# ColumbiaDVMM/ColumbiaImageSearch

Measured on AMD Instinct MI355X. Metric: queries/sec @ recall@10 on 10M LOPQ index, higher is better.
Workload: dtype f64

## Files before the change

columbiaimagesearch_amd/csrc/lopq_scan3.hip:

```cpp
#include "scan_common.h"
#include <cmath>
#include <cstdio>
#include <cstdlib>

typedef unsigned short u16x2_t __attribute__((ext_vector_type(2)));

static __device__ __forceinline__ uint32_t pk_add_u16(uint32_t a, uint32_t b) {
    return __builtin_bit_cast(uint32_t, (u16x2_t)(__builtin_bit_cast(u16x2_t, a) + __builtin_bit_cast(u16x2_t, b)));
}
static __device__ __forceinline__ uint32_t pk_subsat_u16(uint32_t a, uint32_t b) {
    return __builtin_bit_cast(uint32_t, __builtin_elementwise_sub_sat(__builtin_bit_cast(u16x2_t, a), __builtin_bit_cast(u16x2_t, b)));
}

static __device__ __forceinline__ uint32_t pk_min_u16(uint32_t a, uint32_t b) {
    return __builtin_bit_cast(uint32_t, __builtin_elementwise_min(__builtin_bit_cast(u16x2_t, a), __builtin_bit_cast(u16x2_t, b)));
}

static const int S3G = 4;

#ifdef CIS_S3_COUNTERS
__device__ unsigned long long g_s3_ctr[16];
#define S3_CLK() ((long long)__builtin_amdgcn_s_memtime())
#define S3_CTR(i, v) do { if (threadIdx.x == 0) atomicAdd(&g_s3_ctr[i], (unsigned long long)(v)); } while (0)
extern "C" int cis_debug_counters3(unsigned long long* out, int reset) {
// ... 557 lines not shown
                const uint32_t sg = (g & 1) ? (d[u][g >> 1] >> 16) : (d[u][g >> 1] & 0xffffu);
                const uint32_t t1 = (g & 1) ? ((g >> 1) ? s23 >> 16 : s01 >> 16) : ((g >> 1) ? s23 & 0xffffu : s01 & 0xffffu);
                pm[u][g] = __ballot(sg < t1) & anym[u];
                if (any_dup) {
                    bool same = true;
#pragma unroll
                    for (int i = 0; i < (M + 3) / 4; ++i) same = same && (cur[u].w[i] == dup[g].w[i]);
                    pm[u][g] &= ~(__ballot(same) & (has_dup[g] ? ~0ull : 0ull));
                }
            }
        }
#pragma unroll
        for (int g = 0; g < G; ++g) {
            if (g >= ng) break;
            uint32_t* rk = rk_all + (g * NW + w) * R;
            int ntot = 0;
#pragma unroll
            for (int u = 0; u < U; ++u) ntot += __popcll(pm[u][g]);
            if (ntot == 0) continue;
            auto entry = [&](int u) -> uint32_t {
                const uint32_t sg = (g & 1) ? (d[u][g >> 1] >> 16) : (d[u][g >> 1] & 0xffffu);
                return (sg << 16) | (uint32_t)(base + u * 64 + lane);
            };
            if (cnt[g] + ntot <= R) {
                int c = cnt[g];
#pragma unroll
                for (int u = 0; u < U; ++u) {
                    const unsigned long long m = pm[u][g];
                    if (m == 0ull) continue;
                    const int idx = __builtin_amdgcn_mbcnt_hi((unsigned)(m >> 32), __builtin_amdgcn_mbcnt_lo((unsigned)m, c));
                    if ((m >> lane) & 1ull) rk[idx] = entry(u);
                    c += __popcll(m);
                }
                cnt[g] = c;
                continue;
            }
            int u0 = 0;
            while (true) {
                bool full = false;
#pragma unroll
                for (int u = 0; u < U; ++u) {
                    const unsigned long long m = pm[u][g];
                    if (u < u0 || full || m == 0ull) continue;
                    const int n = __popcll(m);
                    if (cnt[g] + n > R) {
                        full = true;
                        u0 = u;
                        continue;
                    }
                    const int idx = cnt[g] + __builtin_amdgcn_mbcnt_hi((unsigned)(m >> 32), __builtin_amdgcn_mbcnt_lo((unsigned)m, 0));
                    if ((m >> lane) & 1ull) rk[idx] = entry(u);
                    cnt[g] += n;
                    u0 = u + 1;
                }
                if (!full) break;
                const QScale qsg = load_scale(&sh[g]);
                int c2 = wave_compact3<M, NR, NW>(rk, cnt[g], L, Lw, R - 64, qsg, &sh[g], w);
                if (c2 < 0) {
                    uint32_t dp = 0xffffffffu;
                    const WorkItem itg = items[item_idx[g]];
                    c2 = wave_compact3_exact<M, NR, NW>(rk, cnt[g], L, Lw, qsg, &sh[g], w, codes, start, K,
                                                        T + (int64_t)itg.tab0 * nf * K, T + (int64_t)itg.tab1 * nf * K, dp);
                    dp = (uint32_t)__builtin_amdgcn_readfirstlane((int)dp);
                    if (dp != 0xffffffffu) {
                        dup[g] = load_code<M>(codes, start + (int64_t)dp);
                        has_dup[g] = true;
                        any_dup = true;
                    }
                }
                cnt[g] = c2;
                const uint32_t thg = lds_ld(&sh[g].thr);
                if (lane == 0) st16(&thr1[g], thg + 1u);
                const unsigned long long dup_on = has_dup[g] ? ~0ull : 0ull;
#pragma unroll
                for (int u = 0; u < U; ++u) {
                    const uint32_t sg = (g & 1) ? (d[u][g >> 1] >> 16) : (d[u][g >> 1] & 0xffffu);
                    bool same = true;
#pragma unroll
                    for (int i = 0; i < (M + 3) / 4; ++i) same = same && (cur[u].w[i] == dup[g].w[i]);
                    pm[u][g] &= __ballot(sg <= thg) & ~(__ballot(same) & dup_on);
                }
            }
        }
    }
    S3_CTR(4, S3_CLK() - c0);
#pragma unroll
    for (int g = 0; g < G; ++g) {
        if (g >= ng) break;
        uint32_t* rk = rk_all + (g * NW + w) * R;
        if (cnt[g] > 0) cnt[g] = wave_compact3<M, NR, NW>(rk, cnt[g], L, Lw, NR * 64, load_scale(&sh[g]), &sh[g], w);
    }
    S3_CTR(5, S3_CLK() - c0);
    if constexpr (NW > 1) __syncthreads();
    S3_CTR(6, S3_CLK() - c0);
#pragma unroll
    for (int g = 0; g < G; ++g) {
        if (g >= ng) break;
        uint32_t* rk = rk_all + (g * NW + w) * R;
        const QScale qsg = load_scale(&sh[g]);
        if constexpr (NW > 1) cnt[g] = wave_filter3<NR, NW>(rk, cnt[g], qsg, &sh[g]);
        if (lane == 0) sh[g].wcnt[w] = cnt[g];
        if (tid == 0) {
            const uint64_t b = block_bound<NW>(&sh[g]);
            if (b < sh[g].ext) atomicMin(&qbound[items[item_idx[g]].q], (unsigned long long)b);
        }
    }
    if constexpr (NW > 1) __syncthreads();
#pragma unroll
    for (int g = 0; g < G; ++g) {
        if (g >= ng) break;
        const uint32_t* rk = rk_all + (g * NW + w) * R;
        int off = 0, total = 0;
#pragma unroll
        for (int i = 0; i < NW; ++i) {
            const int c = (NW > 1) ? sh[g].wcnt[i] : cnt[g];
            off += (i < w) ? c : 0;
            total += c;
        }
        uint64_t* out = item_surv + (int64_t)item_idx[g] * S + off;
        for (int e = lane; e < cnt[g]; e += 64) {
            const uint32_t x = rk[e];
            out[e] = ((uint64_t)(x >> 16) << 32) | (x & 0xffffu);
        }
        if (tid == 0) item_n[item_idx[g]] = total;
    }
    S3_CTR(7, S3_CLK() - c0);
    S3_CTR(0, 1);
}

template <int M, int NR, int U, int NW, int WPE>
__global__ __launch_bounds__(NW * 64) __attribute__((amdgpu_waves_per_eu(WPE, WPE))) void k_adc_scan3(
    const WorkItem* __restrict__ items, const TabDesc* __restrict__ tabs, const int* __restrict__ slots,
    const int* __restrict__ n_slots_ptr, const double* __restrict__ T, const float* __restrict__ T32,
    const uint8_t* __restrict__ codes, int K, int L, int S, int* __restrict__ queue_ctr ,
    uint64_t* __restrict__ item_surv, int* __restrict__ item_n, float* __restrict__ item_slack,
    unsigned long long* __restrict__ qbound , int two_pass, int single_queue ) {
    extern __shared__ __attribute__((aligned(16))) char smem[];
    constexpr int G = S3G;
    constexpr int R = NR * 64 - 8;
    int* s_next = reinterpret_cast<int*>(smem + (size_t)K * M * G * 2 + (size_t)G * NW * R * 4 + G * sizeof(Scan3Shared) + 32);
    const int* qs = n_slots_ptr + 8;
    const int home = blockIdx.x & 7;
    const long long k0 = S3_CLK();
    (void)k0;
    for (int a = 0; a < 8; ++a) {
        const int x = (home + a) & 7;
        const int qstart = qs[x];
        const int count = single_queue ? (x == 0 ? qs[1] - qstart : 0) : qs[x + 1] - qstart;
        if (count <= 0) continue;
        while (true) {
            const long long q0 = S3_CLK();
            (void)q0;
            int j;
            if constexpr (NW > 1) {
                __syncthreads();
                if (threadIdx.x == 0) *s_next = atomicAdd(&queue_ctr[x], 1);
                __syncthreads();
                j = __builtin_amdgcn_readfirstlane(*s_next);
            } else {
                int t = 0;
                if (threadIdx.x == 0) t = atomicAdd(&queue_ctr[x], 1);
                j = __builtin_amdgcn_readfirstlane(t);
            }
            S3_CTR(8, S3_CLK() - q0);
            if (j >= count) break;
            const int slot = qstart + j;
            int idx[G];
            int ng = 0;
            bool same = true;
#pragma unroll
            for (int g = 0; g < G; ++g) {
                idx[g] = slots[slot * G + g];
                if (idx[g] >= 0) {
                    ng = g + 1;
                    same = same && items[idx[g]].start == items[idx[0]].start && items[idx[g]].len == items[idx[0]].len;
                } else {
                    idx[g] = idx[0];
                }
            }
            if (!same) {
                for (int g2 = 0; g2 < ng; ++g2) {
                    int oi[G];
#pragma unroll
                    for (int g = 0; g < G; ++g) {
                        oi[g] = idx[0];
#pragma unroll
                        for (int gg = 1; gg < G; ++gg)
                            if (gg == g2) oi[g] = idx[gg];
                    }
                    if (g2 > 0) __syncthreads();
                    scan3_group<M, NR, U, NW>(items, tabs, oi, 1, T, T32, codes, K, L, S, item_surv, item_n, item_slack, qbound, smem, two_pass != 0);
                }
                continue;
            }
            scan3_group<M, NR, U, NW>(items, tabs, idx, ng, T, T32, codes, K, L, S, item_surv, item_n, item_slack, qbound, smem, two_pass != 0);
        }
    }
    S3_CTR(9, S3_CLK() - k0);
    S3_CTR(10, 1);
}

struct Slot4 {
    int item[S3G], tab0[S3G], tab1[S3G], q[S3G];
    float qinv[S3G];
    int start_lo, start_hi, len, ng;
    int ist_lo[S3G], ist_hi[S3G], ilen[S3G];
};
struct Scan4Shared {
    double inv_up, ub;
    uint64_t ext;
    uint32_t tau;
    int verify;
    int cnt;
    int q;
};

template <int M, int UU, int OCT = (M >= 8 ? 8 : 4), bool TWO = false>
__device__ __forceinline__ void adc16_rows(const CodeWords<M> (&cur)[UU], const RotConsts<M>& rc, const Adc16Consts<M, TWO>& gc,
                                           u32x2_t (&d)[UU]) {
    constexpr int NU = M / OCT;
    u32x2_t fbuf[2][OCT];
    uint32_t D[2][(M + 3) / 4];
    rot_words<M>(cur[0], rc, D[0]);
    adc16_issue<M, OCT, TWO>(D[0], 0, gc, fbuf[0]);
#pragma unroll
    for (int q = 0; q < UU * NU; ++q) {
        const int u = q / NU, o = q % NU;
        if (q + 1 < UU * NU) {
            const int u1 = (q + 1) / NU, o1 = (q + 1) % NU;
            if (o1 == 0) rot_words<M>(cur[u1], rc, D[u1 & 1]);
            adc16_issue<M, OCT, TWO>(D[u1 & 1], o1, gc, fbuf[(q + 1) & 1]);
        }
        __builtin_amdgcn_sched_barrier(0);
        const u32x2_t part = adc16_sum<OCT>(fbuf[q & 1]);
        if (o == 0) {
            d[u] = part;
        } else {
            d[u][0] = pk_add_u16(d[u][0], part[0]);
            d[u][1] = pk_add_u16(d[u][1], part[1]);
        }
        __builtin_amdgcn_sched_barrier(0);
    }
}

static __device__ __forceinline__ void lds_barrier() {
    asm volatile("s_waitcnt lgkmcnt(0)\n\ts_barrier" ::: "memory");
}

#ifndef CIS_S4_U
#define CIS_S4_U 2
#endif
#ifndef CIS_S4_UL
#define CIS_S4_UL 2
#endif
#ifndef CIS_S4_OCT
#define CIS_S4_OCT 4
#endif
#ifndef CIS_S4_WPE
#define CIS_S4_WPE 6
#endif
static const int S4_OCT = CIS_S4_OCT;
#ifndef CIS_S4_PF
#define CIS_S4_PF 2
#endif
#ifndef CIS_S4_LCAP
#define CIS_S4_LCAP 504
#endif
#ifndef CIS_S4_NS
#define CIS_S4_NS 16
#endif
#ifndef CIS_S4_Z
#define CIS_S4_Z 4.0f
#endif
static const int S4_DS = 8;
static const int S4_LCAP = CIS_S4_LCAP;
static const int S4_NS = CIS_S4_NS;

static const int S4_LCAP_LONG = 1016;

static const int S4_TWO_NRP = 24;
static constexpr bool scan4_two(int M, int lcap) { return M == 8 && lcap > 504; }
static constexpr size_t scan4_two_tab(int K, int lcap) {
    const size_t t = (size_t)K * 8 * S3G * 4, l = (((size_t)S3G * lcap + 1) / 2) * 16;
    return t > l ? t : l;
}
static constexpr size_t scan4_two_lds(int K, int lcap, int nw) {
    return scan4_two_tab(K, lcap) + (size_t)S4_TWO_NRP * 128 * 2 + S3G * sizeof(Scan4Shared) + 32 + (size_t)S3G * nw * 4 + (S4_DS + 1) * sizeof(Slot4);
}
static_assert(4 * scan4_two_lds(256, S4_LCAP_LONG, 4) <= 163840, "the two-copy form keeps four workgroups of four waves per CU");
static __device__ __forceinline__ RotConsts<8> two_copy_rot(const RotConsts<8>& rc, uint32_t copy) {
    RotConsts<8> r2 = rc;
#pragma unroll
    for (int t = 0; t < 8; ++t) r2.cj[t] = (rc.cj[t] << 1) | (copy << 2);
    return r2;
}
static __device__ __forceinline__ int two_list_byte(int i) { return ((i >> 1) << 4) + ((i & 1) << 2) + 8; }

static size_t scan4_lds(int M, int K, int lcap, int nw) {
    if (scan4_two(M, lcap)) return scan4_two_lds(K, lcap, nw);
    const size_t lists = (size_t)S3G * lcap * 4, samp = (size_t)S3G * S4_NS * 64 * 2;
    return (size_t)K * M * S3G * 2 + (lists > samp ? lists : samp) + S3G * sizeof(Scan4Shared) + 32 + (size_t)S3G * nw * 4 + (S4_DS + 1) * sizeof(Slot4);
}

static __device__ __forceinline__ int sample_row(int t, int nrows, int ns) { return (int)(((uint32_t)t * (uint32_t)nrows) / (uint32_t)ns); }

template <int M, int U, int NW, int WPE, int LCAPT>
__global__ __launch_bounds__(NW * 64) __attribute__((amdgpu_waves_per_eu(WPE, WPE))) void k_adc_scan4(
    const WorkItem* __restrict__ items, const TabDesc* __restrict__ tabs, const int* __restrict__ slots,
    const int* __restrict__ n_slots_ptr, const float* __restrict__ T32 , const double* __restrict__ T,
    const uint8_t* __restrict__ codes, int K, int L, int S,
    int* __restrict__ dbg , int* __restrict__ fhdr ,
    int* __restrict__ fslots, uint64_t* __restrict__ item_surv, int* __restrict__ item_n, float* __restrict__ item_slack,
    unsigned long long* __restrict__ qbound, float zq , int frac_den ,
    int nsx , int dyn ,
    float sat ) {
    extern __shared__ __attribute__((aligned(16))) char smem[];
    constexpr int G = S3G;
    static_assert(NW >= G && NW % G == 0 && NW <= 8, "waves 0 .. G-1 serve one query each in the threshold and verification phases");
    static_assert(M == 4 || M == 8 || M == 16, "float4s of the half tables are dealt to the threads in rounds of 256");
    constexpr int nf = M / 2;
    constexpr uint32_t CAP = 65535u / M;
    constexpr int LCAP = LCAPT, NS = S4_NS, NRV = (LCAP + 63) / 64;
    constexpr size_t LIST_B_FULL = (size_t)G * LCAP * 4 > (size_t)G * NS * 64 * 2 ? (size_t)G * LCAP * 4 : (size_t)G * NS * 64 * 2;
    constexpr bool TWO = scan4_two(M, LCAPT);
    constexpr size_t LIST_B = TWO ? (size_t)S4_TWO_NRP * 128 * 2 : LIST_B_FULL;
    static_assert(!TWO || LIST_B >= (size_t)NW * 64 * 8, "the bucket minima of the sample fit the position lists' region");
    char* tab = smem;
    uint32_t* lists = reinterpret_cast<uint32_t*>(smem + (TWO ? scan4_two_tab(K, LCAPT) : (size_t)K * M * G * 2));
    uint16_t* samp = reinterpret_cast<uint16_t*>(lists);
    Scan4Shared* sh = reinterpret_cast<Scan4Shared*>(reinterpret_cast<char*>(lists) + LIST_B);
    uint16_t* thr1 = reinterpret_cast<uint16_t*>(sh + G);
    int* s_flag = reinterpret_cast<int*>(thr1 + 4);
    int* s_cnt = s_flag + 1;
    int* wcnt = reinterpret_cast<int*>(reinterpret_cast<char*>(thr1) + 32);
    Slot4* sd = reinterpret_cast<Slot4*>(reinterpret_cast<char*>(thr1) + 32 + G * NW * 4);
    constexpr int WCAP = LCAPT / NW;
    constexpr int PCAP_LDS = (int)(LIST_B / (NW * 2));
    constexpr int NRP = (TWO ? S4_TWO_NRP : (LCAPT > 504 ? 32 : 16)) / NW;
    constexpr int PCAP = NRP * 128 < PCAP_LDS ? NRP * 128 : PCAP_LDS;
    static_assert(PCAP % 2 == 0 && (PCAP_LDS * 2) % 4 == 0, "position lists are read back as 32-bit pairs");
    const int tid = threadIdx.x, lane = tid & 63;
    const int w = __builtin_amdgcn_readfirstlane(tid >> 6);
    const int total = n_slots_ptr[0];
    const int xcd = blockIdx.x & 7, lb = blockIdx.x >> 3;
    const int LW = gridDim.x >> 3;
    auto slot_of = [&](int k) -> int {
        const int li = lb + k * LW;
        const int j = (((li >> 5) * 8 + xcd) << 5) | (li & 31);
        return j < total ? j : -1;
    };
    RotConsts<M> rc = make_rot<M>(lane);
    if constexpr (TWO) rc = two_copy_rot(rc, ((uint32_t)lane >> 3) & 1u);
    const Adc16Consts<M, TWO> gc = adc16_consts<M, TWO>(rc, tab);
    auto list_at = [&](int i) -> uint32_t* { return reinterpret_cast<uint32_t*>(tab + two_list_byte(i)); };
    const int nvec = (nf * K) >> 2;
    const long long k0 = S3_CLK();
    (void)k0;
    for (int kb = 0;; kb += S4_DS) {
        int dyn_j = -1;
        if (LCAPT > 504 && dyn) {
            __syncthreads();
            if (tid == 0) {
                int jn = -1;
                if (dyn == 1) {
                    jn = atomicAdd(&dbg[6], 1);
                    jn = jn < total ? jn : -1;
                } else {
                    int* qx = dbg - 9;
                    for (int a2 = 0; a2 < 8 && jn < 0; ++a2) {
                        const int x = (xcd + a2) & 7;
                        const int li = atomicAdd(&qx[x], 1);
                        const int jj = (((li >> 5) * 8 + x) << 5) | (li & 31);
                        if (jj < total) jn = jj;
                    }
                }
                *s_flag = jn;
            }
            __syncthreads();
            dyn_j = *s_flag;
            if (dyn_j < 0) break;
        } else {
            if (slot_of(kb) < 0) break;
        }
        __syncthreads();
        if (tid < S4_DS) {
            Slot4 d;
            int dyn_s = dyn;
            asm volatile("" : "+s"(dyn_s));
            const int j = (LCAPT > 504 && dyn_s) ? (tid == 0 ? dyn_j : -1) : slot_of(kb + tid);
            d.ng = 0; d.len = 0; d.start_lo = d.start_hi = 0;
#pragma unroll
            for (int g = 0; g < G; ++g) { d.item[g] = 0; d.tab0[g] = 0; d.tab1[g] = 0; d.q[g] = 0; d.qinv[g] = 0.f; d.ist_lo[g] = d.ist_hi[g] = d.ilen[g] = 0; }
            if (j >= 0) {
                int idx[G];
                int ng = 0;
                bool same = true;
#pragma unroll
                for (int g = 0; g < G; ++g) idx[g] = slots[j * G + g];
                const int64_t st0 = items[idx[0]].start;
                const int len0 = items[idx[0]].len;
#pragma unroll
                for (int g = 0; g < G; ++g) {
                    if (idx[g] >= 0) ng = g + 1;
                    else idx[g] = idx[0];
                    const WorkItem* it = &items[idx[g]];
                    same = same && it->start == st0 && it->len == len0;
                    const int t0 = it->tab0, t1 = it->tab1;
                    d.item[g] = idx[g]; d.tab0[g] = t0; d.tab1[g] = t1; d.q[g] = it->q;
                    d.ist_lo[g] = (int)(uint32_t)it->start; d.ist_hi[g] = (int)(it->start >> 32); d.ilen[g] = it->len;
                    float mxT = fmaxf(__int_as_float(tabs[t0].pad), __int_as_float(tabs[t1].pad));
                    mxT = fmaxf(mxT, 1e-30f);
                    float qi = ((float)CAP / mxT) * (1.0f - 9.5367431640625e-7f);
                    qi = (mxT < 3.0e38f) ? qi : 0.0f;
                    qi = (qi < 3.0e38f) ? qi : 3.0e38f;
                    d.qinv[g] = qi;
                }
                d.start_lo = (int)(uint32_t)st0; d.start_hi = (int)(st0 >> 32); d.len = len0;
                d.ng = same ? ng : -ng;
            }
            int tid_d = tid;
            asm volatile("" : "+v"(tid_d));
            sd[tid_d] = d;
        }
        __syncthreads();
        for (int kk = 0; kk < S4_DS; ++kk) {
            const Slot4* d = &sd[kk];
            const int ngs0 = __builtin_amdgcn_readfirstlane(d->ng);
            if (ngs0 == 0) break;
            int remaining = ngs0 < 0 ? ((1 << (-ngs0)) - 1) : 0;
            do {
            if (ngs0 < 0) {
                Slot4* ds = &sd[S4_DS];
                if (tid == 0) {
                    const Slot4* src = &sd[kk];
                    int g0 = 0;
                    while (!((remaining >> g0) & 1)) ++g0;
                    int n = 0, rest = remaining;
                    for (int h = g0; h < G; ++h) {
                        if (((remaining >> h) & 1) && src->ist_lo[h] == src->ist_lo[g0] && src->ist_hi[h] == src->ist_hi[g0] && src->ilen[h] == src->ilen[g0]) {
                            ds->item[n] = src->item[h]; ds->tab0[n] = src->tab0[h]; ds->tab1[n] = src->tab1[h]; ds->q[n] = src->q[h];
                            ds->qinv[n] = src->qinv[h];
                            ++n;
                            rest &= ~(1 << h);
                        }
                    }
                    for (int h = n; h < G; ++h) {
                        ds->item[h] = ds->item[0]; ds->tab0[h] = ds->tab0[0]; ds->tab1[h] = ds->tab1[0]; ds->q[h] = ds->q[0]; ds->qinv[h] = ds->qinv[0];
                    }
                    ds->start_lo = src->ist_lo[g0]; ds->start_hi = src->ist_hi[g0]; ds->len = src->ilen[g0];
                    ds->ng = n;
                    ds->ist_lo[0] = rest;
                }
                lds_barrier();
                d = ds;
                remaining = __builtin_amdgcn_readfirstlane(ds->ist_lo[0]);
            }
            const int ngs = __builtin_amdgcn_readfirstlane(d->ng);
            const long long c0 = S3_CLK();
            (void)c0;
            const int ng = ngs;
            bool fail = false;
            if (!fail) {
                float qinv[G];
#pragma unroll
                for (int g = 0; g < G; ++g)
                    qinv[g] = __builtin_bit_cast(float, __builtin_amdgcn_readfirstlane(__builtin_bit_cast(int, d->qinv[g])));
                const int len = __builtin_amdgcn_readfirstlane(d->len);
                const int64_t start = ((int64_t)__builtin_amdgcn_readfirstlane(d->start_hi) << 32) | (uint32_t)__builtin_amdgcn_readfirstlane(d->start_lo);
                if (sat > 0.0f) {
                    if (w < G) {
                        const int g = w;
                        if (g < ng) {
                            const int t0 = __builtin_amdgcn_readfirstlane(d->tab0[g]), t1 = __builtin_amdgcn_readfirstlane(d->tab1[g]);
                            const int64_t Ta = (int64_t)t0 * nf * K, Tb = (int64_t)t1 * nf * K;
                            const int c = len >= 64 ? (int)(((int64_t)lane * len) >> 6) : lane;
                            uint32_t key = 0x7f7fffffu;
                            if (c < len) {
                                const CodeWords<M> cw = load_code<M>(codes, start + c);
                                float ds = 0.f;
#pragma unroll
                                for (int j = 0; j < M / 2; ++j) ds += tab_f1(T32, T, Ta + j * K + ((cw.w[j >> 2] >> (8 * (j & 3))) & 255u));
#pragma unroll
                                for (int j = 0; j < M / 2; ++j) ds += tab_f1(T32, T, Tb + j * K + ((cw.w[(M / 2 + j) >> 2] >> (8 * ((M / 2 + j) & 3))) & 255u));
                                key = __float_as_uint(fmaxf(ds, 0.f));
                            }
                            int rk = 4 + (int)((64 * (int64_t)L + len - 1) / len);
                            rk = rk > 48 ? 48 : rk;
                            uint32_t mn = key;
                            for (int r = 0; r < rk; ++r) {
                                uint32_t mx = 0u;
                                mn = key;
                                wave_minmax_step<1>(mn, mx); wave_minmax_step<2>(mn, mx); wave_minmax_step<4>(mn, mx);
                                wave_minmax_step<8>(mn, mx); wave_minmax_step<16>(mn, mx); wave_minmax_step<32>(mn, mx);
                                if (r + 1 < rk) {
                                    const uint64_t hit = __ballot(key == mn);
                                    if (lane == (int)__builtin_ctzll(hit)) key = 0x7f7fffffu;
                                }
                            }
                            const float d4 = __uint_as_float(mn);
                            const float qs = (sat * (float)CAP) / fmaxf(d4, 1e-30f);
                            const float q0 = d->qinv[g];
                            if (lane == 0 && q0 > 0.0f && qs > q0 && qs < 3.0e38f && d4 < 1.0e38f) const_cast<Slot4*>(d)->qinv[g] = qs;
                        }
                    }
                    lds_barrier();
#pragma unroll
                    for (int g = 0; g < G; ++g)
                        qinv[g] = __builtin_bit_cast(float, __builtin_amdgcn_readfirstlane(__builtin_bit_cast(int, d->qinv[g])));
                }
                int tid_st = tid;
                asm volatile("" : "+v"(tid_st));
                for (int vt = tid_st; vt < nvec; vt += NW * 64) {
                    const int j = vt & (nf - 1), kq = vt / nf, k0 = 4 * kq;
                    const int vidx = j * (K >> 2) + kq;
                    float4 pv[G][2];
#pragma unroll
                    for (int g = 0; g < G; ++g) {
                        const int t0 = __builtin_amdgcn_readfirstlane(d->tab0[g]), t1 = __builtin_amdgcn_readfirstlane(d->tab1[g]);
                        pv[g][0] = tab_f4(T32, T, t0, nf * K, vidx);
                        pv[g][1] = tab_f4(T32, T, t1, nf * K, vidx);
                    }
                    uint32_t* tw = reinterpret_cast<uint32_t*>(tab);
#pragma unroll
                    for (int s2 = 0; s2 < 2; ++s2) {
#pragma unroll
                        for (int c = 0; c < 4; ++c) {
                            uint32_t qv[G];
#pragma unroll
                            for (int g = 0; g < G; ++g) {
                                const float4 q = pv[g][s2];
                                const float x = c == 0 ? q.x : (c == 1 ? q.y : (c == 2 ? q.z : q.w));
                                qv[g] = (g < ng) ? (uint32_t)(x * qinv[g]) : CAP;
                                qv[g] = qv[g] > CAP ? CAP : qv[g];
                            }
                            u32x2_t pk;
                            pk[0] = qv[0] | (qv[1] << 16);
                            pk[1] = qv[2] | (qv[3] << 16);
                            if constexpr (TWO) {
                                u32x4_t pk2;
                                pk2[0] = pk[0]; pk2[1] = pk[1]; pk2[2] = pk[0]; pk2[3] = pk[1];
                                *reinterpret_cast<u32x4_t*>(tw + (((k0 + c) * M + s2 * nf + j) << 2)) = pk2;
                            } else {
                                *reinterpret_cast<u32x2_t*>(tw + (((k0 + c) * M + s2 * nf + j) << 1)) = pk;
                            }
                        }
                    }
                }
                if (tid >= 64 && tid < 64 + G) {
                    const int g = tid - 64;
                    float qi = qinv[0];
#pragma unroll
                    for (int gg = 1; gg < G; ++gg) qi = (g == gg) ? qinv[gg] : qi;
                    const double inv_up = (double)qi * (1.0 + 2.384185791015625e-7);
                    const double ub = qi > 0.0f ? (1.0 + 4.76837158203125e-7) / (double)qi : __longlong_as_double(0x7ff0000000000000LL);
                    const int item = d->item[g];
                    const int q = d->q[g];
                    sh[g].inv_up = inv_up;
                    sh[g].ub = ub;
                    sh[g].q = q;
                    sh[g].ext = (g < ng) ? __hip_atomic_load(&qbound[q], __ATOMIC_RELAXED, __HIP_MEMORY_SCOPE_AGENT) : 0x7ff0000000000000ull;
                    sh[g].cnt = 0;
                    s_cnt[g] = 0;
                    if (g < ng) {
                        item_slack[2 * (int64_t)item + 0] = __double2float_ru(ub * ((double)M + 0.1));
                        item_slack[2 * (int64_t)item + 1] = __double2float_ru(ub);
                    }
                }
                if (tid == 0) *s_flag = 0;
                __amdgpu_buffer_rsrc_t rs;
                {
                    const uint64_t cbase = (uint64_t)(uintptr_t)(codes + start * M);
                    const uint32_t blo = (uint32_t)__builtin_amdgcn_readfirstlane((int)(uint32_t)cbase);
                    const uint32_t bhi = (uint32_t)__builtin_amdgcn_readfirstlane((int)(uint32_t)(cbase >> 32));
                    rs = __builtin_amdgcn_make_buffer_rsrc((void*)(uintptr_t)(((uint64_t)bhi << 32) | blo), 0, len * M, 0x00020000);
                }
                const int nrows = (len + 63) >> 6;
                constexpr bool MULTI = LCAPT > 504;
                if constexpr (!MULTI) {
                    const int ns = nrows < NS ? nrows : NS;
                    constexpr int SPW = NS / NW;
                    static_assert(NS % (2 * NW) == 0, "sample rows come in pairs per wave");
                    CodeWords<M> sc[SPW];
                    int srow[SPW];
#pragma unroll
                    for (int i = 0; i < SPW; ++i) {
                        const int t = SPW * w + i;
                        srow[i] = t < ns ? sample_row(t, nrows, ns) : nrows;
                        sc[i] = load_code_buf<M>(rs, srow[i] * 64 + lane);
                    }
                    S3_CTR(11, S3_CLK() - c0);
                    lds_barrier();
                    S3_CTR(2, S3_CLK() - c0);
                    {
                        u32x2_t dd[SPW];
                        adc16_rows<M, SPW, S4_OCT>(sc, rc, gc, dd);
#pragma unroll
                        for (int u = 0; u < SPW; ++u) {
                            const int t = SPW * w + u;
                            const bool ok = (t < ns) && (srow[u] * 64 + lane < len);
#pragma unroll
                            for (int g = 0; g < G; ++g) {
                                const uint32_t sg = (g & 1) ? (dd[u][g >> 1] >> 16) : (dd[u][g >> 1] & 0xffffu);
                                samp[g * (NS * 64) + t * 64 + lane] = (uint16_t)(ok ? sg : 0xffffu);
                            }
                        }
                    }
                    lds_barrier();
                    S3_CTR(3, S3_CLK() - c0);
                    if (w < G) {
                        const int g = w;
                        uint32_t sv[NS];
                        int nsam = 0;
#pragma unroll
                        for (int r = 0; r < NS; ++r) {
                            sv[r] = samp[g * (NS * 64) + r * 64 + lane];
                            nsam += __popcll(__ballot(sv[r] != 0xffffu));
                        }
                        const bool exact = ns == nrows;
                        int ksv = L;
                        if (!exact) {
                            const float need = (float)L * (float)nsam / (float)len;
                            float zq_s = zq;
                            asm volatile("" : "+s"(zq_s));
                            const float hz = 0.5f * zq_s;
                            const float rt = hz + sqrtf(hz * hz + need);
                            ksv = (int)(rt * rt) + 1;
                        }
                        uint32_t tau = 65534u;
                        bool have_bound = false;
                        if (g < ng && nsam >= ksv) {
                            uint32_t lo = 0u, hi = 65534u;
                            while (lo < hi) {
                                const uint32_t p = lo + ((hi - lo) >> 1);
                                int c = 0;
#pragma unroll
                                for (int r = 0; r < NS; ++r) c += __popcll(__ballot(sv[r] <= p));
                                if (c >= ksv) hi = p;
                                else lo = p + 1;
                            }
                            tau = lo;
                            have_bound = tau < (sat > 0.f ? CAP - (uint32_t)M - 2u : 65534u);
                        }
                        if (lane == 0) {
                            uint32_t keep = 65534u;
                            if (have_bound) {
                                keep = tau + (uint32_t)M + 1u;
                                keep = keep < 65534u ? keep : 65534u;
                            }
                            const uint32_t t_ext = (g < ng) ? bound_to_thr(sh[g].ext, sh[g].inv_up) : 0u;
                            const uint32_t t = keep < t_ext ? keep : t_ext;
                            thr1[g] = (uint16_t)((g < ng) ? t + 1u : 0u);
                            sh[g].tau = tau;
                            sh[g].verify = (have_bound && keep < t_ext && !exact) ? 1 : 0;
                        }
                    }
                } else {
                    int ns = nrows / frac_den;
                    ns = ns < NS ? NS : ns;
                    ns = ns > nsx ? nsx : ns;
                    ns = ns < nrows ? ns : nrows;
                    constexpr int SPW = 4;
                    const int rounds = (ns + NW * SPW - 1) / (NW * SPW);
                    CodeWords<M> sc[SPW];
                    int srow[SPW];
#pragma unroll
                    for (int i = 0; i < SPW; ++i) {
                        const int t = SPW * w + i;
                        srow[i] = t < ns ? sample_row(t, nrows, ns) : nrows;
                        sc[i] = load_code_buf<M>(rs, srow[i] * 64 + lane);
                    }
                    S3_CTR(11, S3_CLK() - c0);
                    lds_barrier();
                    S3_CTR(2, S3_CLK() - c0);
                    {
                        uint32_t bm0 = 0xffffffffu, bm1 = 0xffffffffu;
#pragma unroll 1
                        for (int r = 0; r < rounds; ++r) {
                            CodeWords<M> nsc[SPW];
                            int nrow[SPW];
                            if constexpr (MULTI) {
                                if (r + 1 < rounds) {
#pragma unroll
                                    for (int i = 0; i < SPW; ++i) {
                                        const int t = ((r + 1) * NW + w) * SPW + i;
                                        nrow[i] = t < ns ? sample_row(t, nrows, ns) : nrows;
                                        nsc[i] = load_code_buf<M>(rs, nrow[i] * 64 + lane);
                                    }
                                }
                            }
                            u32x2_t dd[SPW];
                            adc16_rows<M, SPW, S4_OCT, TWO>(sc, rc, gc, dd);
#pragma unroll
                            for (int u = 0; u < SPW; ++u) {
                                const bool ok = srow[u] < nrows && (srow[u] * 64 + lane < len);
                                bm0 = pk_min_u16(bm0, ok ? dd[u][0] : 0xffffffffu);
                                bm1 = pk_min_u16(bm1, ok ? dd[u][1] : 0xffffffffu);
                            }
                            if constexpr (MULTI) {
                                if (r + 1 < rounds) {
#pragma unroll
                                    for (int i = 0; i < SPW; ++i) { sc[i] = nsc[i]; srow[i] = nrow[i]; }
                                }
                            }
                        }
                        u32x2_t bm;
                        bm[0] = bm0; bm[1] = bm1;
                        reinterpret_cast<u32x2_t*>(samp)[w * 64 + lane] = bm;
                    }
                    lds_barrier();
                    S3_CTR(3, S3_CLK() - c0);
                    if (w < G) {
                        const int g = w;
                        uint32_t sv[NW];
#pragma unroll
                        for (int r = 0; r < NW; ++r) {
                            const uint32_t xw = lds_ld(reinterpret_cast<const uint32_t*>(samp) + 2 * (r * 64 + lane) + (g >> 1));
                            sv[r] = (g & 1) ? (xw >> 16) : (xw & 0xffffu);
                        }
                        const bool all = ns == nrows;
                        const int nsam = all ? len : ns * 64;
                        int ksv = L;
                        if (!all) {
                            const float need = (float)L * (float)nsam / (float)len;
                            const float hz = 0.5f * zq;
                            const float rt = hz + sqrtf(hz * hz + need);
                            ksv = (int)(rt * rt) + 1;
                        }
                        uint32_t tau = 65534u;
                        bool have_bound = false;
                        if (g < ng && nsam >= ksv) {
                            uint32_t lo = 0u, hi = 65534u;
                            while (lo < hi) {
                                const uint32_t p = lo + ((hi - lo) >> 1);
                                int c = 0;
#pragma unroll
                                for (int r = 0; r < NW; ++r) c += __popcll(__ballot(sv[r] <= p));
                                if (c >= ksv) hi = p;
                                else lo = p + 1;
                            }
                            tau = lo;
                            have_bound = tau < (sat > 0.f ? CAP - (uint32_t)M - 2u : 65534u);
                        }
                        if (lane == 0) {
                            uint32_t keep = 65534u;
                            if (have_bound) {
                                keep = tau + (uint32_t)M + 1u;
                                keep = keep < 65534u ? keep : 65534u;
                            }
                            const uint32_t t_ext = (g < ng) ? bound_to_thr(sh[g].ext, sh[g].inv_up) : 0u;
                            const uint32_t t = keep < t_ext ? keep : t_ext;
                            thr1[g] = (uint16_t)((g < ng) ? t + 1u : 0u);
                            sh[g].tau = tau;
                            sh[g].verify = (have_bound && keep < t_ext && !all) ? 1 : 0;
                        }
                    }
                }
                lds_barrier();
                S3_CTR(4, S3_CLK() - c0);
                {
                    const uint64_t tp64 = lds_ld(reinterpret_cast<const uint64_t*>(thr1));
                    u32x2_t tpk;
                    tpk[0] = (uint32_t)tp64; tpk[1] = (uint32_t)(tp64 >> 32);
                    const uint32_t s01 = (uint32_t)__builtin_amdgcn_readfirstlane((int)tpk[0]);
                    const uint32_t s23 = (uint32_t)__builtin_amdgcn_readfirstlane((int)tpk[1]);
                    const int nit = (len + 64 * U - 1) / (64 * U);
                    constexpr int PF = CIS_S4_PF;
                    CodeWords<M> ring[PF][U];
#pragma unroll
                    for (int k = 0; k < PF; ++k) {
#pragma unroll
                        for (int u = 0; u < U; ++u) ring[k][u] = load_code_buf<M>(rs, (w + k * NW) * 64 * U + u * 64 + lane);
                        __builtin_amdgcn_sched_barrier(0);
                    }
                    int wcur[G];
#pragma unroll
                    for (int g = 0; g < G; ++g) wcur[g] = 0;
                    uint16_t* plist = reinterpret_cast<uint16_t*>(lists) + (size_t)w * PCAP_LDS;
                    int pcur = 0;
                    for (int iter0 = w; iter0 < nit; iter0 += NW * PF) {
#pragma unroll
                      for (int k = 0; k < PF; ++k) {
                        const int iter = iter0 + k * NW;
                        const int base = iter * 64 * U;
                        u32x2_t dd[U];
                        adc16_rows<M, U, S4_OCT, TWO>(ring[k], rc, gc, dd);
#pragma unroll
                        for (int u = 0; u < U; ++u) ring[k][u] = load_code_buf<M>(rs, (iter + PF * NW) * 64 * U + u * 64 + lane);
#pragma unroll
                        for (int u = 0; u < U; ++u) {
                            const uint32_t xx = pk_subsat_u16(tpk[0], dd[u][0]) | pk_subsat_u16(tpk[1], dd[u][1]);
                            const int n = len - base - u * 64;
                            if constexpr (TWO) {
                                const bool pass = xx != 0u && lane < n;
                                const unsigned long long am = __builtin_amdgcn_ballot_w64(xx != 0u) & __builtin_amdgcn_ballot_w64(lane < n);
                                if (am == 0ull) continue;
                                const int idx = __builtin_amdgcn_mbcnt_hi((unsigned)(am >> 32), __builtin_amdgcn_mbcnt_lo((unsigned)am, pcur));
                                if (pass && idx < PCAP) plist[idx] = (uint16_t)(base + u * 64 + lane);
                                pcur += __popcll(am);
                                continue;
                            }
                            unsigned long long am = __ballot(xx != 0u);
                            if (n < 64) am &= n <= 0 ? 0ull : ((1ull << n) - 1ull);
                            if (am == 0ull) continue;
                            const int idx = __builtin_amdgcn_mbcnt_hi((unsigned)(am >> 32), __builtin_amdgcn_mbcnt_lo((unsigned)am, pcur));
                            if (((am >> lane) & 1ull) && idx < PCAP) plist[idx] = (uint16_t)(base + u * 64 + lane);
                            pcur += __popcll(am);
                        }
                      }
                    }
                    S3_CTR(13, S3_CLK() - c0);
                    const bool pover = pcur > PCAP;
                    const int pn = pover ? 0 : pcur;
                    static_assert(NRP * 128 <= PCAP_LDS, "the NRP registers are read from the wave's own position list");
                    uint32_t pp[NRP];
#pragma unroll
                    for (int r = 0; r < NRP; ++r) pp[r] = lds_ld(reinterpret_cast<const uint32_t*>(plist) + r * 64 + lane);
                    auto on_of = [&](int it) -> bool { return 2 * (((it >> 1) * 64) + lane) + (it & 1) < pn; };
                    CodeWords<M> cw[2];
                    cw[0] = load_code_buf<M>(rs, on_of(0) ? (int)(pp[0] & 0xffffu) : len);
                    cw[1] = load_code_buf<M>(rs, on_of(1) ? (int)(pp[0] >> 16) : len);
                    lds_barrier();
                    Adc16Consts<M, TWO> gc0;
                    if constexpr (TWO) {
                        gc0 = gc;
                        uint32_t keep0 = ~8u;
                        asm volatile("" : "+v"(keep0));
#pragma unroll
                        for (int t = 0; t < M; ++t) gc0.c[t] = gc.c[t] & keep0;
                    }
                    if (pn > 0) {
                        const int nreg = (pn + 127) >> 7;
#pragma unroll 1
                        for (int r = 0; r < nreg; ++r) {
                          const uint32_t cur = pp[0];
#pragma unroll
                          for (int k = 0; k + 1 < NRP; ++k) pp[k] = pp[k + 1];
                          pp[NRP - 1] = 0u;
#pragma unroll
                          for (int h = 0; h < 2; ++h) {
                            const int it = 2 * r + h;
                            const uint32_t pos = h ? (cur >> 16) : (cur & 0xffffu);
                            CodeWords<M> cc[1];
                            cc[0] = cw[h];
                            u32x2_t d1[1];
                            if constexpr (TWO) adc16_rows<M, 1, S4_OCT, true>(cc, rc, gc0, d1);
                            else adc16_rows<M, 1, S4_OCT>(cc, rc, gc, d1);
                            cw[h] = load_code_buf<M>(rs, on_of(it + 2) ? (int)(h ? (pp[0] >> 16) : (pp[0] & 0xffffu)) : len);
                            const unsigned long long am2 = __ballot(on_of(it));
#pragma unroll
                            for (int g = 0; g < G; ++g) {
                                const uint32_t sg = (g & 1) ? (d1[0][g >> 1] >> 16) : (d1[0][g >> 1] & 0xffffu);
                                const uint32_t t1 = (g & 1) ? ((g >> 1) ? s23 >> 16 : s01 >> 16) : ((g >> 1) ? s23 & 0xffffu : s01 & 0xffffu);
                                const unsigned long long mg = __ballot(sg < t1) & am2;
                                if (mg == 0ull) continue;
                                const int idx = __builtin_amdgcn_mbcnt_hi((unsigned)(mg >> 32), __builtin_amdgcn_mbcnt_lo((unsigned)mg, wcur[g]));
                                if (((mg >> lane) & 1ull) && idx < WCAP) {
                                    if constexpr (TWO) *list_at((g * NW + w) * WCAP + idx) = (sg << 16) | pos;
                                    else lists[(g * NW + w) * WCAP + idx] = (sg << 16) | pos;
                                }
                                wcur[g] += __popcll(mg);
                            }
                          }
                        }
                    }
                    if (pover) wcur[0] = WCAP + 1;
                    if (lane < G) {
                        int c = wcur[0];
#pragma unroll
                        for (int g = 1; g < G; ++g) c = (lane == g) ? wcur[g] : c;
                        wcnt[lane * NW + w] = c;
                    }
                }
                S3_CTR(12, S3_CLK() - c0);
                lds_barrier();
                S3_CTR(5, S3_CLK() - c0);
                bool bad = false;
                if (w < ng) {
                    const int g = w;
                    int tot = 0;
                    int wtot[NW];
                    int lane_v = lane;
                    asm volatile("" : "+v"(lane_v));
#pragma unroll
                    for (int r = 0; r < NW; ++r) {
                        wtot[r] = wcnt[g * NW + r];
                        bad = bad || wtot[r] > WCAP;
                        tot += wtot[r];
                    }
                    if (bad && lane_v == 0) atomicAdd(&dbg[2], 1);
                    if (!bad) {
                        uint32_t ent[NRV];
                        bool val[NRV];
#pragma unroll
                        for (int r = 0; r < NRV; ++r) {
                            constexpr int RW = NRV / NW;
                            const int e = (r % RW) * 64 + lane_v;
                            val[r] = e < wtot[r / RW];
                            if constexpr (TWO) ent[r] = val[r] ? *list_at((g * NW + r / RW) * WCAP + e) : 0xffffffffu;
                            else ent[r] = val[r] ? lists[(g * NW + r / RW) * WCAP + e] : 0xffffffffu;
                        }
                        const uint32_t tau = sh[g].tau;
                        if (sh[g].verify) {
                            int nle = 0;
#pragma unroll
                            for (int r = 0; r < NRV; ++r) nle += __popcll(__ballot(val[r] && (ent[r] >> 16) <= tau));
                            bad = nle < L;
                            if (bad && lane_v == 0) atomicAdd(&dbg[3], 1);
                        }
                        if (!bad) {
                            uint32_t cut = 65535u;
                            if (tot >= L) {
                                uint32_t mn = 0xffffffffu, mx = 0u;
#pragma unroll
                                for (int r = 0; r < NRV; ++r) {
                                    const uint32_t s = ent[r] >> 16;
                                    mn = (val[r] && s < mn) ? s : mn;
                                    mx = (val[r] && s > mx) ? s : mx;
                                }
                                wave_minmax_all(mn, mx);
                                uint32_t lo = mn, hi = mx;
                                while (lo < hi) {
                                    const uint32_t p = lo + ((hi - lo) >> 1);
                                    int c = 0;
#pragma unroll
                                    for (int r = 0; r < NRV; ++r) c += __popcll(__ballot(val[r] && (ent[r] >> 16) <= p));
                                    if (c >= L) {
                                        hi = p;
                                        if (c <= L + 16) break;
                                    } else {
                                        lo = p + 1;
                                    }
                                }
                                cut = hi + (uint32_t)M + 1u;
                                if (sat > 0.f && cut >= CAP) {
                                    bad = true;
                                    if (lane_v == 0) atomicAdd(&dbg[4], 1);
                                }
                                const uint64_t b = val_to_bound(hi, M, sh[g].ub);
                                if (lane_v == 0 && !bad && b < sh[g].ext) atomicMin(&qbound[sh[g].q], (unsigned long long)b);
                            } else if (sat > 0.f) {
                                bool sat = false;
#pragma unroll
                                for (int r = 0; r < NRV; ++r) sat = sat || (__ballot(val[r] && (ent[r] >> 16) + (uint32_t)M + 1u >= CAP) != 0ull);
                                if (sat) {
                                    bad = true;
                                    if (lane_v == 0) atomicAdd(&dbg[4], 1);
                                }
                            }
                            const int item = __builtin_amdgcn_readfirstlane(d->item[g]);
                            uint64_t* out = item_surv + (int64_t)item * S;
                            if constexpr (LCAP > 504) {
                                int nk = 0;
#pragma unroll
                                for (int r = 0; r < NRV; ++r) nk += __popcll(__ballot(val[r] && (ent[r] >> 16) <= cut));
                                if (nk > S) {
                                    bad = true;
                                    if (lane_v == 0) atomicAdd(&dbg[4], 1);
                                }
                            }
                            if (!bad) {
                                int kept = 0;
#pragma unroll
                                for (int r = 0; r < NRV; ++r) {
                                    const bool kp = val[r] && (ent[r] >> 16) <= cut;
                                    const unsigned long long mk = __ballot(kp);
                                    const int idx = kept + __builtin_amdgcn_mbcnt_hi((unsigned)(mk >> 32), __builtin_amdgcn_mbcnt_lo((unsigned)mk, 0));
                                    if (kp) out[idx] = ((uint64_t)(ent[r] >> 16) << 32) | (ent[r] & 0xffffu);
                                    kept += __popcll(mk);
                                }
                                if (lane_v == 0) item_n[item] = kept;
                            }
                        }
                    }
                    if (bad && lane_v == 0) *s_flag = 1;
                }
                lds_barrier();
                S3_CTR(6, S3_CLK() - c0);
                fail = *s_flag != 0;
            }
            S3_CTR(0, 1);
            if (tid == 0) {
                atomicAdd(&dbg[0], 1);
                if (ngs0 < 0) atomicAdd(&dbg[5], 1);
                if (fail) {
                    atomicAdd(&dbg[1], 1);
                    const int f = atomicAdd(&fhdr[17], 1);
#pragma unroll
                    for (int g = 0; g < G; ++g) fslots[f * G + g] = g < ng ? d->item[g] : -1;
                }
            }
            } while (remaining != 0);
        }
    }
    S3_CTR(9, S3_CLK() - k0);
    S3_CTR(10, 1);
}

template <int M, int NR>
static void launch_scan3_k(const Scan3Geom& g, const ScanArgs& a, bool fallback) {
    constexpr int U = 4, NW = 4;
    constexpr int WPE = M == 16 ? 3 : 4;
    const int by_lds = (int)(163840 / g.lds), by_waves = (WPE * 4) / NW;
    const unsigned grid = fallback ? 256u : persistent_grid(a, g.G, by_lds < by_waves ? by_lds : by_waves);
    hipLaunchKernelGGL((k_adc_scan3<M, NR, U, NW, WPE>), dim3(grid), dim3(NW * 64), g.lds, a.st, a.items, a.tabs, fallback ? a.fslots : a.slots,
                       fallback ? a.fhdr + 8 : a.n_slots, a.T, a.T32, a.codes, a.K, a.L, g.S, fallback ? a.fhdr : a.qctr, a.hits, a.hitn, a.slack, a.qbound,
                       fallback ? (g.long_chunks ? 0 : 1) : g.two_pass, fallback ? 1 : 0);
}

bool scan3_supported(int M, int K, int L) {
    return (M == 4 || M == 8 || M == 16) && K <= 256 && K % 4 == 0 && L >= 1 && L <= 440;
}

Scan3Geom scan3_geom(int M, int K, int L, int64_t avg_chunk, int force_two_pass) {
    Scan3Geom g;
    const int NR = (L <= 184) ? 4 : 8;
    g.G = S3G;
    g.NW = 4;
    (void)avg_chunk;
    g.U = 4;
    g.two_pass = (avg_chunk > 0 && avg_chunk < 12288 && M <= 8) ? 1 : 0;
    if (g.two_pass == 1 && L <= 128 && avg_chunk < 6144) g.two_pass = 2;
    g.long_chunks = avg_chunk >= 6144 ? 1 : 0;
    static const int s4_m16 = getenv("CIS_S4_M16") ? atoi(getenv("CIS_S4_M16")) : 1;
    if (g.two_pass == 0 && g.long_chunks && (M <= 8 || s4_m16) && L <= 128) g.two_pass = 2;
    if (const char* e = getenv("CIS_SCAN3_TWOPASS")) g.two_pass = atoi(e);
    if (force_two_pass >= 0) g.two_pass = force_two_pass;
    if (g.two_pass == 2 && M > 8 && !s4_m16 && force_two_pass != 2) g.two_pass = g.long_chunks ? 0 : 1;
    if (g.two_pass == 1 && g.long_chunks && force_two_pass < 0) g.two_pass = 0;
    if (g.two_pass < 0 || g.two_pass > 2) g.two_pass = 0;
    g.S = g.NW * (NR * 64 - 8);
    g.lds = (size_t)K * M * g.G * 2 + (size_t)g.G * g.NW * (NR * 64 - 8) * 4 + g.G * sizeof(Scan3Shared) + 32 + 16;
    return g;
}

template <int M, int U, int NW, int WPE, int LCAP>
static void launch_scan4(const Scan3Geom& g, const ScanArgs& a, float z, int frac, int sample_rows, int dyn) {
    const size_t lds = scan4_lds(M, a.K, LCAP, NW);
    const int by_lds = (int)(163840 / lds), by_waves = (WPE * 4) / NW;
    int per_cu = by_lds < by_waves ? by_lds : by_waves;
    if (const char* e = getenv("CIS_S4_PER_CU")) per_cu = atoi(e) > 0 && atoi(e) < per_cu ? atoi(e) : per_cu;
    hipLaunchKernelGGL((k_adc_scan4<M, U, NW, WPE, LCAP>), dim3(persistent_grid(a, g.G, per_cu)), dim3(NW * 64), lds, a.st, a.items, a.tabs, a.slots, a.n_slots, a.T32, a.T,
                       a.codes, a.K, a.L, g.S, a.qctr + 9, a.fhdr, a.fslots, a.hits, a.hitn, a.slack, a.qbound, z, frac, sample_rows, dyn, g.sat);
}

template <int M, int NR>
static void launch_scan3_t(const Scan3Geom& g, const ScanArgs& a) {
    if (g.two_pass != 2) {
        launch_scan3_k<M, NR>(g, a, false);
        return;
    }
    const float z_short = getenv("CIS_S4_ZS") ? (float)atof(getenv("CIS_S4_ZS")) : CIS_S4_Z;
    const float z_long = getenv("CIS_S4_ZL") ? (float)atof(getenv("CIS_S4_ZL")) : 4.5f;
    const int frac_long = getenv("CIS_S4_FRAC") ? atoi(getenv("CIS_S4_FRAC")) : 8;
    const int nsx_long = getenv("CIS_S4_NSX") ? atoi(getenv("CIS_S4_NSX")) : 128;
    const int dyn_long = getenv("CIS_S4_DYN") ? atoi(getenv("CIS_S4_DYN")) : 0;
    if (!g.long_chunks) {
        constexpr int WPE4 = (M == 16) ? 4 : CIS_S4_WPE;
        launch_scan4<M, CIS_S4_U, 4, WPE4, S4_LCAP>(g, a, z_short, 1 << 20, S4_NS, 0);
    } else {
        constexpr int WPE4 = (M == 16) ? 3 : 4;
        launch_scan4<M, CIS_S4_UL, 4, WPE4, S4_LCAP_LONG>(g, a, z_long, frac_long, nsx_long, dyn_long);
    }
    if (getenv("CIS_SCAN4_DEBUG")) {
        int h[6] = {0, 0, 0, 0, 0, 0};
        if (hipMemcpyAsync(h, a.qctr + 9, sizeof(h), hipMemcpyDeviceToHost, a.st) == hipSuccess && hipStreamSynchronize(a.st) == hipSuccess)
            fprintf(stderr, "[cis] k_adc_scan4: %d slots, %d to the fall-back list (lists: %d overflowed, %d failed the verification, %d crowds at the cut; %d slots with items of different chunks)\n",
                    h[0], h[1], h[2], h[3], h[4], h[5]);
    }
    launch_scan3_k<M, NR>(g, a, true);
}

void launch_scan3(int M, const Scan3Geom& g, const ScanArgs& a) {
    dispatch_int<4, 8, 16>(M, [&](auto m) { dispatch_nr<8>(a.L, [&](auto nr) { launch_scan3_t<decltype(m)::value, decltype(nr)::value>(g, a); }); });
}
```

Measured before the change: 26.11 million.

## Deepen sample-row prefetch ring and issue scan code loads before threshold phase

The multi-round sampling loop becomes a 4-deep ring of 2-row sets with loads issued ahead. For M<=8 the main scan's code prefetch ring is now issued before the threshold/barrier phase, so its latency overlaps threshold selection. The sample-row index division is replaced by a multiply-high with a precomputed reciprocal, and an unused shared counter is dropped. The cost is more live registers for the early ring and the sample ring, which may hurt occupancy under the fixed waves-per-EU bound.

```diff
diff --git a/columbiaimagesearch_amd/csrc/lopq_scan3.hip b/columbiaimagesearch_amd/csrc/lopq_scan3.hip
--- a/columbiaimagesearch_amd/csrc/lopq_scan3.hip
+++ b/columbiaimagesearch_amd/csrc/lopq_scan3.hip
@@ -883,7 +883,10 @@
     return (size_t)K * M * S3G * 2 + (lists > samp ? lists : samp) + S3G * sizeof(Scan4Shared) + 32 + (size_t)S3G * nw * 4 + (S4_DS + 1) * sizeof(Slot4);
 }
 
-static __device__ __forceinline__ int sample_row(int t, int nrows, int ns) { return (int)(((uint32_t)t * (uint32_t)nrows) / (uint32_t)ns); }
+static __device__ __forceinline__ uint32_t sample_inv(int ns) { return 0x7fffffffu / (uint32_t)ns + 1u; }
+static __device__ __forceinline__ int sample_row(int t, int nrows, int ns, uint32_t inv) {
+    return (int)__umulhi(2u * (uint32_t)(t < ns ? t : ns) * (uint32_t)nrows, inv);
+}
 
 template <int M, int U, int NW, int WPE, int LCAPT>
 __global__ __launch_bounds__(NW * 64) __attribute__((amdgpu_waves_per_eu(WPE, WPE))) void k_adc_scan4(
@@ -912,7 +915,6 @@
     Scan4Shared* sh = reinterpret_cast<Scan4Shared*>(reinterpret_cast<char*>(lists) + LIST_B);
     uint16_t* thr1 = reinterpret_cast<uint16_t*>(sh + G);
     int* s_flag = reinterpret_cast<int*>(thr1 + 4);
-    int* s_cnt = s_flag + 1;
     int* wcnt = reinterpret_cast<int*>(reinterpret_cast<char*>(thr1) + 32);
     Slot4* sd = reinterpret_cast<Slot4*>(reinterpret_cast<char*>(thr1) + 32 + G * NW * 4);
     constexpr int WCAP = LCAPT / NW;
@@ -1141,7 +1143,6 @@
                     sh[g].q = q;
                     sh[g].ext = (g < ng) ? __hip_atomic_load(&qbound[q], __ATOMIC_RELAXED, __HIP_MEMORY_SCOPE_AGENT) : 0x7ff0000000000000ull;
                     sh[g].cnt = 0;
-                    s_cnt[g] = 0;
                     if (g < ng) {
                         item_slack[2 * (int64_t)item + 0] = __double2float_ru(ub * ((double)M + 0.1));
                         item_slack[2 * (int64_t)item + 1] = __double2float_ru(ub);
@@ -1157,16 +1158,28 @@
                 }
                 const int nrows = (len + 63) >> 6;
                 constexpr bool MULTI = LCAPT > 504;
+                constexpr int PF = CIS_S4_PF;
+                constexpr bool RING_EARLY = M <= 8;
+                CodeWords<M> ring[PF][U];
+                auto ring_first = [&]() {
+#pragma unroll
+                    for (int k = 0; k < PF; ++k) {
+#pragma unroll
+                        for (int u = 0; u < U; ++u) ring[k][u] = load_code_buf<M>(rs, (w + k * NW) * 64 * U + u * 64 + lane);
+                        __builtin_amdgcn_sched_barrier(0);
+                    }
+                };
                 if constexpr (!MULTI) {
                     const int ns = nrows < NS ? nrows : NS;
                     constexpr int SPW = NS / NW;
                     static_assert(NS % (2 * NW) == 0, "sample rows come in pairs per wave");
                     CodeWords<M> sc[SPW];
                     int srow[SPW];
+                    const uint32_t sinv = sample_inv(ns);
 #pragma unroll
                     for (int i = 0; i < SPW; ++i) {
                         const int t = SPW * w + i;
-                        srow[i] = t < ns ? sample_row(t, nrows, ns) : nrows;
+                        srow[i] = sample_row(t, nrows, ns, sinv);
                         sc[i] = load_code_buf<M>(rs, srow[i] * 64 + lane);
                     }
                     S3_CTR(11, S3_CLK() - c0);
@@ -1186,6 +1199,7 @@
                             }
                         }
                     }
+                    if constexpr (RING_EARLY) ring_first();
                     lds_barrier();
                     S3_CTR(3, S3_CLK() - c0);
                     if (w < G) {
@@ -1241,14 +1255,24 @@
                     ns = ns > nsx ? nsx : ns;
                     ns = ns < nrows ? ns : nrows;
                     constexpr int SPW = 4;
-                    const int rounds = (ns + NW * SPW - 1) / (NW * SPW);
-                    CodeWords<M> sc[SPW];
-                    int srow[SPW];
-#pragma unroll
-                    for (int i = 0; i < SPW; ++i) {
-                        const int t = SPW * w + i;
-                        srow[i] = t < ns ? sample_row(t, nrows, ns) : nrows;
-                        sc[i] = load_code_buf<M>(rs, srow[i] * 64 + lane);
+                    constexpr int SRS = 2;
+                    constexpr int SD = 4;
+                    static_assert(SPW % SRS == 0, "a set does not straddle rounds");
+                    const uint32_t sinv = sample_inv(ns);
+                    auto t_of = [&](int j) -> int { return ((j / SPW) * NW + w) * SPW + (j % SPW); };
+                    int rows_w = ns % (NW * SPW) - SPW * w;
+                    rows_w = (ns / (NW * SPW)) * SPW + (rows_w < 0 ? 0 : (rows_w > SPW ? SPW : rows_w));
+                    const int nsets = (rows_w + SRS - 1) / SRS;
+                    CodeWords<M> sring[SD][SRS];
+                    int srow[SD][SRS];
+#pragma unroll
+                    for (int k = 0; k < SD; ++k) {
+#pragma unroll
+                        for (int i = 0; i < SRS; ++i) {
+                            srow[k][i] = sample_row(t_of(k * SRS + i), nrows, ns, sinv);
+                            sring[k][i] = load_code_buf<M>(rs, srow[k][i] * 64 + lane);
+                        }
+                        __builtin_amdgcn_sched_barrier(0);
                     }
                     S3_CTR(11, S3_CLK() - c0);
                     lds_barrier();
@@ -1256,34 +1280,28 @@
                     {
                         uint32_t bm0 = 0xffffffffu, bm1 = 0xffffffffu;
 #pragma unroll 1
-                        for (int r = 0; r < rounds; ++r) {
-                            CodeWords<M> nsc[SPW];
-                            int nrow[SPW];
-                            if constexpr (MULTI) {
-                                if (r + 1 < rounds) {
-#pragma unroll
-                                    for (int i = 0; i < SPW; ++i) {
-                                        const int t = ((r + 1) * NW + w) * SPW + i;
-                                        nrow[i] = t < ns ? sample_row(t, nrows, ns) : nrows;
-                                        nsc[i] = load_code_buf<M>(rs, nrow[i] * 64 + lane);
+                        for (int s0 = 0; s0 < nsets; s0 += SD) {
+#pragma unroll
+                            for (int k = 0; k < SD; ++k) {
+                                const int st = s0 + k;
+                                if (st < nsets) {
+                                    u32x2_t dd[SRS];
+                                    adc16_rows<M, SRS, S4_OCT, TWO>(sring[k], rc, gc, dd);
+#pragma unroll
+                                    for (int u = 0; u < SRS; ++u) {
+                                        const bool ok = srow[k][u] * 64 + lane < len;
+                                        bm0 = pk_min_u16(bm0, ok ? dd[u][0] : 0xffffffffu);
+                                        bm1 = pk_min_u16(bm1, ok ? dd[u][1] : 0xffffffffu);
                                     }
                                 }
-                            }
-                            u32x2_t dd[SPW];
-                            adc16_rows<M, SPW, S4_OCT, TWO>(sc, rc, gc, dd);
-#pragma unroll
-                            for (int u = 0; u < SPW; ++u) {
-                                const bool ok = srow[u] < nrows && (srow[u] * 64 + lane < len);
-                                bm0 = pk_min_u16(bm0, ok ? dd[u][0] : 0xffffffffu);
-                                bm1 = pk_min_u16(bm1, ok ? dd[u][1] : 0xffffffffu);
-                            }
-                            if constexpr (MULTI) {
-                                if (r + 1 < rounds) {
-#pragma unroll
-                                    for (int i = 0; i < SPW; ++i) { sc[i] = nsc[i]; srow[i] = nrow[i]; }
+#pragma unroll
+                                for (int i = 0; i < SRS; ++i) {
+                                    srow[k][i] = sample_row(t_of((st + SD) * SRS + i), nrows, ns, sinv);
+                                    sring[k][i] = load_code_buf<M>(rs, srow[k][i] * 64 + lane);
                                 }
                             }
                         }
+                        if constexpr (RING_EARLY) ring_first();
                         u32x2_t bm;
                         bm[0] = bm0; bm[1] = bm1;
                         reinterpret_cast<u32x2_t*>(samp)[w * 64 + lane] = bm;
@@ -1345,14 +1363,7 @@
                     const uint32_t s01 = (uint32_t)__builtin_amdgcn_readfirstlane((int)tpk[0]);
                     const uint32_t s23 = (uint32_t)__builtin_amdgcn_readfirstlane((int)tpk[1]);
                     const int nit = (len + 64 * U - 1) / (64 * U);
-                    constexpr int PF = CIS_S4_PF;
-                    CodeWords<M> ring[PF][U];
-#pragma unroll
-                    for (int k = 0; k < PF; ++k) {
-#pragma unroll
-                        for (int u = 0; u < U; ++u) ring[k][u] = load_code_buf<M>(rs, (w + k * NW) * 64 * U + u * 64 + lane);
-                        __builtin_amdgcn_sched_barrier(0);
-                    }
+                    if constexpr (!RING_EARLY) ring_first();
                     int wcur[G];
 #pragma unroll
                     for (int g = 0; g < G; ++g) wcur[g] = 0;
```

After: 26.53 million (median of 6 runs). +1.6%, better.
